# cwfparsonson/ddls

Hardware: AMD Instinct MI355X
Metric: ppo_env_steps_per_sec (higher is better)
Workload: dtype fp32; 1 GPU; model=pacml_gnn_msg32_hidden64_2rounds, global_batch=4096, seq_len=150, parallelism=dp1, ramp=4x4x2_32workers, envs_per_rank=256, env_engine=gpu_resident, num_sgd_iter=50, sgd_minibatch_size=128

## Files before the change

ddls_amd/ops/hip/cached_step.hip:

```cpp
#include <hip/hip_runtime.h>
#include <torch/extension.h>
#include <ATen/cuda/CUDAContext.h>
#include <cstdlib>
#include <cstring>
#include <vector>

#include "cs_stage.h"

#define LN_EPS 1e-5f

#define FMA(a, b, c) __builtin_fmaf((a), (b), (c))
__device__ __forceinline__ float mul_rn(float a, float b) {
  float p = a * b;
  asm("" : "+v"(p));
  return p;
}

#define KF0 5
#define KFE 2
#define KH 16
#define KMSG 32
#define KHID 64
#define KOUT 16
#define KGF 34
// ... 1709 lines not shown
      const float surr1 = ratio * A_b, surr2 = r_cl * A_b;
      float ds = ratio * A_b;
      if (surr2 < surr1 && (ratio < 1.f - D.clip || ratio > 1.f + D.clip))
        ds = 0.f;
      const float coef = -ds - klc;
      P.hent[b] = ent;
      P.coef[b] = coef;
      sHent[s] = ent;
      sCoef[s] = coef;
    }
    __syncthreads();
    for (int x = tid; x < ns * KA; x += NT) {
      const int s = x / KA, a = x % KA;
      const int b = c0 + s;
      const long u = (long)b * KA + a;
      const long act = P.actions[b];
      const float c = sCoef[s] / D.B;
      const float pj = sPp[s][a];
      const float lpj = sLp[s][a];
      P.p[u] = pj;
      P.lp[u] = lpj;
      const float delta = (a == (int)act) ? 1.f : 0.f;
      const float gl = mul_rn(c, delta - pj)
                       + mul_rn(mul_rn(D.ent_coef / D.B, pj),
                                lpj + sHent[s]);
      P.glogits[u] = gl;
      sGL[s][a] = gl;
    }
    if (tid >= 128 && tid < 128 + ns) {
      const int s = tid - 128;
      const int b = c0 + s;
      const float verr = sVal[s] - P.vtarg[b];
      const float mk = (verr * verr <= D.vf_clip) ? 1.f : 0.f;
      const float gv = D.vf_coef * 2.f * verr * mk / D.B;
      P.gvalue[b] = gv;
      sGV[s] = gv;
    }
    __syncthreads();
#pragma unroll
    for (int s = 0; s < HS; ++s) {
      if (s < ns) {
        const int j = tid;
        const long u = (long)(c0 + s) * KFC + j;
        float acc = 0.f;
#pragma unroll
        for (int a = 0; a < KA; ++a) {
          const float w = sW2p[a * HD_ROW + hd_pad(j)];
          if (a < 5) acc = FMA(w, sGL[s][a], acc);
          else acc = acc + mul_rn(w, sGL[s][a]);
        }
        const float gp = hp[s] > 0.f ? acc : 0.f;
        const float av = w2v * sGV[s];
        const float gv = hv[s] > 0.f ? av : 0.f;
        P.gh1p[u] = gp;
        P.gh1v[u] = gv;
        sGHp[s][j] = gp;
        sGHv[s][j] = gv;
      }
    }
    __syncthreads();
    for (int x = tid; x < ns * KFIN; x += NT) {
      const int s = x / KFIN, i = x % KFIN;
      float acc = 0.f;
#pragma unroll 8
      for (int j = 0; j < KFC; ++j) {
        acc = FMA(sW1p[j * KFIN + i], sGHp[s][j], acc);
        acc = FMA(sW1v[j * KFIN + i], sGHv[s][j], acc);
      }
      P.gfinal[(long)(c0 + s) * KFIN + i] = acc;
      sGF[s][i] = acc;
    }
    __syncthreads();
    for (int x = tid; x < ns * KGF; x += NT) {
      const int s = x / KGF, i = x % KGF;
      float acc = 0.f;
#pragma unroll
      for (int o = 0; o < KGE; ++o)
        acc = acc + mul_rn(sWg[o * KGF + i], sGF[s][KOUT + o]);
      P.gu34[(long)(c0 + s) * KGF + i] = acc;
    }
  }
}

__global__ void __launch_bounds__(256)
cs_fwd_comb2_pool_kernel(CachedPtrs P, CachedDims D) {
  constexpr int PT = 256;
  __shared__ float sH2[PT * KOUT];
  const int tid = threadIdx.x;
  const int m = blockIdx.x;
  const long lo = P.model_nptr[m], hi = P.model_nptr[m + 1];
  float acc = 0.f;
  for (long v0 = lo; v0 < hi; v0 += PT) {
    const long v1 = min(hi, v0 + PT);
    __syncthreads();
    for (long x = tid; x < (v1 - v0) * KOUT; x += 256) {
      const long v = v0 + x / KOUT;
      const int i = (int)(x % KOUT);
      const long qlo = P.indptr[v], qhi = P.indptr[v + 1];
      float out = 0.f;
      if (qhi > qlo) {
        float a = P.rs2[v * KOUT + i];
        for (long q = qlo; q < qhi; ++q)
          a = a + P.re2[P.order[q] * KOUT + i];
        out = a / (float)(qhi - qlo + 1);
      }
      P.h2[v * KOUT + i] = out;
      sH2[x] = out;
    }
    __syncthreads();
    if (tid < KOUT)
      for (long v = v0; v < v1; ++v) acc = acc + sH2[(v - v0) * KOUT + tid];
  }
  if (tid < KOUT) P.pooled[(long)m * KOUT + tid] = acc / (float)(hi - lo);
}

template <int L>
__global__ void __launch_bounds__(ROW_NT)
cs_fwd_comb1_mlp2_lanes_kernel(CachedPtrs P, CachedDims D) {
  constexpr int RPB = ROW_NT / L;
  const int nbN = (D.N + RPB - 1) / RPB;
  if ((int)blockIdx.x < nbN) {
    const long r0 = (long)blockIdx.x * RPB;
    rows_fwd_lanes<KHID, KH, 0, L>(
        P, W_LN_N2_W, r0, D.N,
        [&](long v, int i) {
          const long lo = P.indptr[v], hi = P.indptr[v + 1];
          float out = 0.f;
          if (hi > lo) {
            float acc = P.rs1[v * KHID + i];
            for (long q = lo; q < hi; ++q)
              acc = acc + P.re1[P.order[q] * KHID + i];
            out = acc / (float)(hi - lo + 1);
          }
          P.h1[v * KHID + i] = out;
          return out;
        },
        P.xh_h2, P.rst_h2, P.hn2);
  } else {
    const long r0 = (long)(blockIdx.x - nbN) * RPB;
    rows_fwd_lanes<KFE, KH, 0, L>(
        P, W_LN_E2_W, r0, D.E,
        [&](long k, int i) { return P.e[k * KFE + i]; },
        P.xh_e2, P.rst_e2, P.he2);
  }
}

template <int L>
__global__ void __launch_bounds__(ROW_NT)
cs_bwd_scat2_mlp2_lanes_kernel(CachedPtrs P, CachedDims D) {
  constexpr int RPB = ROW_NT / L;
  const int nbN = (D.N + RPB - 1) / RPB;
  if ((int)blockIdx.x < nbN) {
    const long r0 = (long)blockIdx.x * RPB;
    rows_bwd_lanes<KHID, KH, KH, 0, L, true>(
        P, W_LN_N2_W, r0, D.N,
        [&](long v, int o) {
          const long lo = P.src_indptr[v], hi = P.src_indptr[v + 1];
          float acc = P.gms2[v * KMSG + o];
          for (long q = lo; q < hi; ++q)
            acc = acc + P.gme2[P.src_order[q] * KMSG + o];
          P.ghn2[v * KH + o] = acc;
          return acc;
        },
        P.hn2, P.xh_h2, P.rst_h2, P.gpn1, P.gu_h2, P.gh1b);
  } else {
    const long r0 = (long)(blockIdx.x - nbN) * RPB;
// ... 385 lines not shown
          }
        }
#pragma unroll
        for (int q = 0; q < MYU2; ++q) {
          int u = tid + q * NT;
          if (u < KA * JW) {
            int a = u / JW, j = u % JW;
            float s = acc2[q];
            if (rt == TILE_K) {
#pragma unroll
              for (int t = 0; t < TILE_K; ++t) {
                if (t < 20) s = FMA(tGL[r0 + t][a], tHp[r0 + t][j], s);
                else s = s + mul_rn(tGL[r0 + t][a], tHp[r0 + t][j]);
              }
            } else {
              for (int t = 0; t < rt; ++t)
                s = FMA(tGL[r0 + t][a], tHp[r0 + t][j], s);
            }
            acc2[q] = s;
          }
        }
      }
      if (cj >= 0 && cj < JW) {
        if (st == WFC_ST) {
#pragma unroll 16
          for (int t = 0; t < WFC_ST; ++t) {
            bp = bp + tGp[t][cj];
            bv = bv + tGv[t][cj];
            w2v = FMA(tGV[t], tHv[t][cj], w2v);
          }
        } else {
          for (int t = 0; t < st; ++t) {
            bp = bp + tGp[t][cj];
            bv = bv + tGv[t][cj];
            w2v = FMA(tGV[t], tHv[t][cj], w2v);
          }
        }
      }
      if (jb == 0) {
        if (tid >= 128 && tid < 128 + KA) {
          if (st == WFC_ST) {
#pragma unroll 16
            for (int t = 0; t < WFC_ST; ++t) b2 = b2 + tGL[t][tid - 128];
          } else {
            for (int t = 0; t < st; ++t) b2 = b2 + tGL[t][tid - 128];
          }
        }
        if (tid == 128 + KA) {
          if (st == WFC_ST) {
#pragma unroll 16
            for (int t = 0; t < WFC_ST; ++t) b2 = b2 + tGV[t];
          } else {
            for (int t = 0; t < st; ++t) b2 = b2 + tGV[t];
          }
        }
      }
      __syncthreads();
    }
#pragma unroll
    for (int q = 0; q < MYU; ++q) {
      int u = tid + q * NT;
      if (u < JW * KFIN) {
        int j = u / KFIN, i = u % KFIN;
        WG_(W_P1_W)[(long)(j0 + j) * KFIN + i] = accp[q];
        WG_(W_V1_W)[(long)(j0 + j) * KFIN + i] = accv[q];
      }
    }
#pragma unroll
    for (int q = 0; q < MYU2; ++q) {
      int u = tid + q * NT;
      if (u < KA * JW) {
        int a = u / JW, j = u % JW;
        WG_(W_P2_W)[(long)a * KFC + j0 + j] = acc2[q];
      }
    }
    if (cj >= 0 && cj < JW) {
      WG_(W_P1_B)[j0 + cj] = bp;
      WG_(W_V1_B)[j0 + cj] = bv;
      WG_(W_V2_W)[j0 + cj] = w2v;
    }
    if (jb == 0) {
      if (tid >= 128 && tid < 128 + KA) WG_(W_P2_B)[tid - 128] = b2;
      if (tid == 128 + KA) WG_(W_V2_B)[0] = b2;
    }
  }
}

static_assert(CS_STAGE_THREADS == ROW_NT, "stage role runs a ROW_NT block");

template <int L>
__global__ void __launch_bounds__(ROW_NT)
cs_fwd_stage_mlp1_lanes_kernel(CachedPtrs P, CachedDims D, StagePtrs SP,
                               StageDims SD) {
  if (blockIdx.x == 0) {
    cs_stage_body(SP, SD);
    return;
  }
  constexpr int RPB = ROW_NT / L;
  const int blk = (int)blockIdx.x - 1;
  const int nbN = (D.N + RPB - 1) / RPB;
  if (blk < nbN) {
    const long r0 = (long)blk * RPB;
    rows_fwd_lanes<KF0, KH, 1, L>(
        P, W_LN_N1_W, r0, D.N,
        [&](long v, int i) { return P.z0[v * KF0 + i]; },
        P.xh_z1, P.rst_z1, P.hn1);
  } else {
    const long r0 = (long)(blk - nbN) * RPB;
    rows_fwd_lanes<KFE, KH, 0, L>(
        P, W_LN_E1_W, r0, D.E,
        [&](long k, int i) { return P.e[k * KFE + i]; },
        P.xh_e1, P.rst_e1, P.he1);
  }
}


template <int Din, int NF>
__device__ __forceinline__ float mod1_elem(
    const float* __restrict__ x, const float* __restrict__ gam,
    const float* __restrict__ bet, const float* __restrict__ w, float b,
    int c, float* __restrict__ xh_c, float* __restrict__ rstd_out) {
  float s = 0.f;
#pragma unroll
  for (int i = 0; i < Din; ++i) s = s + x[i];
  const float mu = s / Din;
  float var;
  {
    const float d0 = x[0] - mu;
    var = d0 * d0;
  }
#pragma unroll
  for (int i = 1; i < Din; ++i) {
    const float d = x[i] - mu;
    if (i >= Din - NF) var = FMA(d, d, var);
    else var = var + d * d;
  }
  float rstd;
  if ((Din & (Din - 1)) == 0) rstd = rsqrtf(FMA(var, 1.f / Din, LN_EPS));
  else rstd = rsqrtf(var / Din + LN_EPS);
  *rstd_out = rstd;
  *xh_c = (x[c] - mu) * rstd;
  float acc = b;
#pragma unroll
  for (int i = 0; i < Din; ++i) {
    const float xh = (x[i] - mu) * rstd;
    acc = FMA(FMA(xh, gam[i], bet[i]), w[i], acc);
  }
  return acc > 0.f ? acc : 0.f;
}

template <int L, bool EDGE>
__device__ __forceinline__ void mlp1_red1_rows(const CachedPtrs& P, long r0,
                                               long nrows) {
  constexpr int RPB = ROW_NT / L;
  constexpr int XS = KMSG + 1;
  constexpr int RW = EDGE ? KF0 + KFE : KF0;
  constexpr int NSM = 2 * KMSG + KHID + (2 * KF0 + KH * KF0 + KH)
                      + (EDGE ? 2 * KFE + KH * KFE + KH : 0);
  constexpr int WQ = KMSG * KHID / ROW_NT;
  static_assert(RPB * RW <= ROW_NT && NSM <= 2 * ROW_NT
                && KMSG * KHID % ROW_NT == 0, "one staging pass");
  __shared__ float sGam[KMSG], sBet[KMSG], sW[KHID * XS], sB[KHID];
  __shared__ float sX[RPB * XS], sU[RPB * XS];
  __shared__ float sM1[2 * KF0 + KH * KF0 + KH + 2 * KFE + KH * KFE + KH];
  __shared__ float sIn[RPB * (KF0 + KFE)];
  float* const sGamN = sM1;
// ... 373 lines not shown
    }
    __syncthreads();
    const int ng = (D.B + SG_SPB - 1) / SG_SPB;
    for (int x = tid; x < ng * 4; x += ROW_NT) {
      const int g = x / 4, k = x % 4;
      const int b_lo = g * SG_SPB;
      const int nb = min(D.B - b_lo, SG_SPB);
      float acc = sT[b_lo][k];
      for (int t = 1; t < nb; ++t) acc = acc + sT[b_lo + t][k];
      sAcc[g][k] = acc;
    }
    __syncthreads();
    if (tid == 0) {
      const float inv = 1.f / D.B;
      const float klc = P.kl[0];
      for (int g = 0; g < ng; ++g) {
        const float pl = sAcc[g][0] * inv;
        const float vf = sAcc[g][1] * inv;
        const float kl = sAcc[g][2] * inv;
        const float ent = sAcc[g][3] * inv;
        atomicAdd(&P.stats[0], pl);
        atomicAdd(&P.stats[1], vf);
        atomicAdd(&P.stats[2], kl);
        atomicAdd(&P.stats[3], ent);
        atomicAdd(&P.stats[4],
                  FMA(-D.ent_coef, ent, FMA(D.vf_coef, vf, FMA(kl, klc, pl))));
      }
    }
  } else if ((int)blockIdx.x < nbN) {
    const long r0 = (long)blockIdx.x * SG_RPB;
    const long v = r0 + r;
    float g = 0.f;
    if (v < D.N) {
      const long lo = P.src_indptr[v], hi = P.src_indptr[v + 1];
      float acc = P.gms1[v * KMSG + i];
      for (long q = lo; q < hi; ++q)
        acc = acc + P.gme1[P.src_order[q] * KMSG + i];
      g = P.hn1[v * KH + i] > 0.f ? acc : 0.f;
      P.ghn1[v * KH + i] = g;
    }
    sG[r][i] = g;
    __syncthreads();
    for (int x = tid; x < SG_RPB * KF0; x += ROW_NT) {
      const int rr = x / KF0, ii = x % KF0;
      if (r0 + rr < D.N) {
        float acc = 0.f;
#pragma unroll
        for (int o = 0; o < KH; ++o)
          acc = FMA(sWN[o * KF0 + ii], sG[rr][o], acc);
        P.gu_z1[(r0 + rr) * KF0 + ii] = acc;
      }
    }
  } else {
    const long r0 = (long)(blockIdx.x - nbN) * SG_RPB;
    const long k = r0 + r;
    float g = 0.f;
    if (k < D.E) {
      const float ge = P.gme1[k * KMSG + KH + i];
      g = P.he1[k * KH + i] > 0.f ? ge : 0.f;
      P.ghe1[k * KH + i] = g;
    }
    sG[r][i] = g;
    __syncthreads();
    for (int x = tid; x < SG_RPB * KFE; x += ROW_NT) {
      const int rr = x / KFE, ii = x % KFE;
      if (r0 + rr < D.E) {
        float acc = 0.f;
#pragma unroll
        for (int o = 0; o < KH; ++o)
          acc = FMA(sWE[o * KFE + ii], sG[rr][o], acc);
        P.gu_e1[(r0 + rr) * KFE + ii] = acc;
      }
    }
  }
}


struct RowCfg {
  bool thread;
  int lanes;
  bool fused;
  bool overlap;
  bool merge;
};

static RowCfg row_cfg() {
  RowCfg c;
  const char* rk = getenv("DDLS_AMD_ROW_KERNELS");
  c.thread = (rk != nullptr && strcmp(rk, "thread") == 0);
  TORCH_CHECK(rk == nullptr || rk[0] == '\0' || c.thread
              || strcmp(rk, "lanes") == 0,
              "cached_step: DDLS_AMD_ROW_KERNELS must be 'thread' or "
              "'lanes', got '", rk, "'");
  c.lanes = 0;
  const char* rl = getenv("DDLS_AMD_ROW_LANES");
  if (rl != nullptr && rl[0] != '\0') {
    c.lanes = atoi(rl);
    TORCH_CHECK(c.lanes == 8 || c.lanes == 16 || c.lanes == 32,
                "cached_step: DDLS_AMD_ROW_LANES must be 8, 16 or 32, got '",
                rl, "'");
  }
  const char* sf = getenv("DDLS_AMD_STEP_FUSION");
  const bool off = (sf != nullptr && strcmp(sf, "off") == 0);
  TORCH_CHECK(sf == nullptr || sf[0] == '\0' || off || strcmp(sf, "on") == 0,
              "cached_step: DDLS_AMD_STEP_FUSION must be 'on' or 'off', got '",
              sf, "'");
  c.fused = !off && !c.thread;
  const char* so = getenv("DDLS_AMD_STEP_OVERLAP");
  const bool ooff = (so != nullptr && strcmp(so, "off") == 0);
  TORCH_CHECK(so == nullptr || so[0] == '\0' || ooff || strcmp(so, "on") == 0,
              "cached_step: DDLS_AMD_STEP_OVERLAP must be 'on' or 'off', got '",
              so, "'");
  c.overlap = !ooff && c.fused;
  const char* sm = getenv("DDLS_AMD_STEP_MERGE");
  const bool moff = (sm != nullptr && strcmp(sm, "off") == 0);
  TORCH_CHECK(sm == nullptr || sm[0] == '\0' || moff || strcmp(sm, "on") == 0,
              "cached_step: DDLS_AMD_STEP_MERGE must be 'on' or 'off', got '",
              sm, "'");
  c.merge = !moff && c.overlap;
  return c;
}

#define LAUNCH_ROWS(KERNEL_L, DEFL, rows0, rows1)                            \
  do {                                                                       \
    const int L_ = R.lanes ? R.lanes : (DEFL);                               \
    const int rpb_ = ROW_NT / L_;                                            \
    const int nb_ = ((rows0) + rpb_ - 1) / rpb_ + ((rows1) + rpb_ - 1) / rpb_; \
    if (nb_ > 0) {                                                           \
      if (L_ == 8)                                                           \
        hipLaunchKernelGGL(KERNEL_L(8), dim3(nb_), dim3(ROW_NT), 0, stream,  \
                           P, D);                                            \
      else if (L_ == 16)                                                     \
        hipLaunchKernelGGL(KERNEL_L(16), dim3(nb_), dim3(ROW_NT), 0, stream, \
                           P, D);                                            \
      else                                                                   \
        hipLaunchKernelGGL(KERNEL_L(32), dim3(nb_), dim3(ROW_NT), 0, stream, \
                           P, D);                                            \
    }                                                                        \
  } while (0)
#define K_FWD_MLP1(L) (cs_fwd_mlp_lanes_kernel<1, L>)
#define K_FWD_MLP2(L) (cs_fwd_mlp_lanes_kernel<2, L>)
#define K_FWD_RED1(L) (cs_fwd_reduce_lanes_kernel<1, L>)
#define K_FWD_RED2(L) (cs_fwd_reduce_lanes_kernel<2, L>)
#define K_BWD_RED1(L) (cs_bwd_reduce_lanes_kernel<1, L>)
#define K_BWD_RED2(L) (cs_bwd_reduce_lanes_kernel<2, L>)
#define K_BWD_MLP2(L) (cs_bwd_mlp2_lanes_kernel<L>)
#define K_FWD_COMB1_MLP2(L) (cs_fwd_comb1_mlp2_lanes_kernel<L>)
#define K_BWD_SCAT2_MLP2(L) (cs_bwd_scat2_mlp2_lanes_kernel<L>)

static void fill_ptrs(CachedPtrs& P, CachedDims& D, RowCfg& R,
                      std::vector<torch::Tensor>& T,
                      std::vector<double>& fs) {
  TORCH_CHECK((int)T.size() == C_NT, "cached_step: tensor list size ",
              T.size(), " != ", (int)C_NT);
  D.N = (int)T[C_Z0].size(0);
  D.F0 = (int)T[C_Z0].size(1);
  D.E = (int)T[C_E].size(0);
  D.FE = (int)T[C_E].size(1);
  D.M = (int)T[C_MODEL_NPTR].size(0) - 1;
  D.B = (int)T[C_GF].size(0);
  D.GFin = (int)T[C_GF].size(1);
  D.A = (int)T[C_MASK].size(1);
  D.H = (int)T[C_HN1].size(1);
  D.MSG = 2 * D.H;
  D.HID = (int)T[C_H1].size(1);
  D.OUT = (int)T[C_H2].size(1);
  D.GEMB = (int)T[C_FINAL].size(1) - D.OUT;
  D.FIN = (int)T[C_FINAL].size(1);
  D.FC = (int)T[C_H1P].size(1);
  const char* wm = getenv("DDLS_AMD_WGRAD_MFMA");
  D.wgrad_mfma = (wm != nullptr && wm[0] == '1') ? 1 : 0;
  R = row_cfg();
  D.clip = (float)fs[0];
  D.vf_clip = (float)fs[1];
  D.vf_coef = (float)fs[2];
  D.ent_coef = (float)fs[3];
  TORCH_CHECK(D.F0 == KF0 && D.FE == KFE && D.H == KH && D.MSG == KMSG
              && D.HID == KHID && D.OUT == KOUT && D.GFin == KGF
              && D.GEMB == KGE && D.FIN == KFIN && D.FC == KFC && D.A == KA,
              "cached_step: compiled for the tuned PAC-ML dims only");
  P.z0 = T[C_Z0].data_ptr<float>();
  P.e = T[C_E].data_ptr<float>();
  P.src = T[C_SRC].data_ptr<long>();
  P.dst = T[C_DST].data_ptr<long>();
  P.order = T[C_ORDER].data_ptr<long>();
  P.indptr = T[C_INDPTR].data_ptr<long>();
  P.src_order = T[C_SRC_ORDER].data_ptr<long>();
  P.src_indptr = T[C_SRC_INDPTR].data_ptr<long>();
  P.node_model = T[C_NODE_MODEL].data_ptr<long>();
  P.model_nptr = T[C_MODEL_NPTR].data_ptr<long>();
  P.model_ids = T[C_MODEL_IDS].data_ptr<long>();
  P.gf = T[C_GF].data_ptr<float>();
  P.mask = T[C_MASK].data_ptr<float>();
  P.actions = T[C_ACTIONS].data_ptr<long>();
  P.old_logp = T[C_OLD_LOGP].data_ptr<float>();
  P.adv = T[C_ADV].data_ptr<float>();
  P.vtarg = T[C_VTARG].data_ptr<float>();
  P.kl = T[C_KL].data_ptr<float>();
  P.flat_p = T[C_FLAT_P].data_ptr<float>();
  P.flat_g = T[C_FLAT_G].data_ptr<float>();
  P.offs = T[C_OFFS].data_ptr<long>();
  P.hn1 = T[C_HN1].data_ptr<float>();
// ... 61 lines not shown
  P.gu_h2 = T[C_GU_H2].data_ptr<float>();
  P.gu_e2 = T[C_GU_E2].data_ptr<float>();
  P.gu_m1e = T[C_GU_M1E].data_ptr<float>();
  P.gu_m1s = T[C_GU_M1S].data_ptr<float>();
  P.gu_z1 = T[C_GU_Z1].data_ptr<float>();
  P.gu_e1 = T[C_GU_E1].data_ptr<float>();
  P.wg_scratch = T[C_WG_SCRATCH].data_ptr<float>();
  TORCH_CHECK(T[C_WG_SCRATCH].numel() >= (long)6 * WSPLIT * WG_JSTRIDE,
              "cached_step: wg_scratch too small");
}

static void step_fwd_launches(const CachedPtrs& P, const CachedDims& D,
                              const RowCfg& R, const StagePtrs* SP,
                              const StageDims* SD) {
  hipStream_t stream = at::cuda::getCurrentCUDAStream();
  const int rows_b = (D.N + D.E + 255) / 256;
  const int comb1_b = ((long)D.N * D.HID + 255) / 256;
  const int comb2_b = ((long)D.N * D.OUT + 255) / 256;
  if (R.thread) {
    hipLaunchKernelGGL(cs_fwd_mlp_kernel<1>, dim3(rows_b), dim3(256), 0,
                       stream, P, D);
    hipLaunchKernelGGL(cs_fwd_reduce_kernel<1>, dim3(rows_b), dim3(256), 0,
                       stream, P, D);
  } else if (R.merge) {
    const int L_ = R.lanes ? R.lanes : 32;
    const int rpb_ = ROW_NT / L_;
    const int stage = SP != nullptr ? 1 : 0;
    const dim3 grid(stage + (D.E + rpb_ - 1) / rpb_ + (D.N + rpb_ - 1) / rpb_);
    StagePtrs sp0;
    StageDims sd0;
    memset(&sp0, 0, sizeof(sp0));
    memset(&sd0, 0, sizeof(sd0));
    const StagePtrs& sp = stage ? *SP : sp0;
    const StageDims& sd = stage ? *SD : sd0;
    if (grid.x > 0) {
      if (L_ == 8)
        hipLaunchKernelGGL(cs_fwd_stage_mlp1_red1_lanes_kernel<8>, grid,
                           dim3(ROW_NT), 0, stream, P, D, sp, sd, stage);
      else if (L_ == 16)
        hipLaunchKernelGGL(cs_fwd_stage_mlp1_red1_lanes_kernel<16>, grid,
                           dim3(ROW_NT), 0, stream, P, D, sp, sd, stage);
      else
        hipLaunchKernelGGL(cs_fwd_stage_mlp1_red1_lanes_kernel<32>, grid,
                           dim3(ROW_NT), 0, stream, P, D, sp, sd, stage);
    }
  } else {
    if (SP != nullptr) {
      const int L_ = R.lanes ? R.lanes : 16;
      const int rpb_ = ROW_NT / L_;
      const dim3 grid(1 + (D.N + rpb_ - 1) / rpb_ + (D.E + rpb_ - 1) / rpb_);
      if (L_ == 8)
        hipLaunchKernelGGL(cs_fwd_stage_mlp1_lanes_kernel<8>, grid,
                           dim3(ROW_NT), 0, stream, P, D, *SP, *SD);
      else if (L_ == 16)
        hipLaunchKernelGGL(cs_fwd_stage_mlp1_lanes_kernel<16>, grid,
                           dim3(ROW_NT), 0, stream, P, D, *SP, *SD);
      else
        hipLaunchKernelGGL(cs_fwd_stage_mlp1_lanes_kernel<32>, grid,
                           dim3(ROW_NT), 0, stream, P, D, *SP, *SD);
    } else {
      LAUNCH_ROWS(K_FWD_MLP1, 16, D.N, D.E);
    }
    LAUNCH_ROWS(K_FWD_RED1, 32, D.E, D.N);
  }
  if (!R.fused)
    hipLaunchKernelGGL(cs_fwd_combine_kernel<1>, dim3(comb1_b), dim3(256), 0,
                       stream, P, D);
  if (R.thread) {
    hipLaunchKernelGGL(cs_fwd_mlp_kernel<2>, dim3(rows_b), dim3(256), 0,
                       stream, P, D);
    hipLaunchKernelGGL(cs_fwd_reduce_kernel<2>, dim3(rows_b), dim3(256), 0,
                       stream, P, D);
  } else {
    if (R.fused)
      LAUNCH_ROWS(K_FWD_COMB1_MLP2, 16, D.N, D.E);
    else
      LAUNCH_ROWS(K_FWD_MLP2, 16, D.N, D.E);
    LAUNCH_ROWS(K_FWD_RED2, 16, D.E, D.N);
  }
  if (R.fused) {
    if (D.M > 0)
      hipLaunchKernelGGL(cs_fwd_comb2_pool_kernel, dim3(D.M), dim3(256), 0,
                         stream, P, D);
    const int hb = D.B < 32 ? D.B : 32;
    if (hb > 0)
      hipLaunchKernelGGL(cs_head_kernel, dim3(hb), dim3(256), 0, stream,
                         P, D);
    return;
  }
  hipLaunchKernelGGL(cs_fwd_combine_kernel<2>, dim3(comb2_b), dim3(256), 0,
                     stream, P, D);
  hipLaunchKernelGGL(cs_fwd_pool_kernel, dim3(1), dim3(512), 0, stream,
                     P, D);
  int head_blocks = ((long)D.B * D.FC + 255) / 256;
  if (head_blocks > 128) head_blocks = 128;
  hipLaunchKernelGGL(cs_fwd_head_kernel, dim3(head_blocks), dim3(256), 0,
                     stream, P, D);
  hipLaunchKernelGGL(cs_fwd_logits_kernel, dim3(D.B), dim3(512), 0,
                     stream, P, D);
  hipLaunchKernelGGL(cs_fwd_loss_kernel, dim3((D.B + 31) / 32), dim3(256),
                     0, stream, P, D);
}

void cached_step_fwd(std::vector<torch::Tensor> T, std::vector<double> fs) {
  CachedPtrs P;
  CachedDims D;
  RowCfg R;
  fill_ptrs(P, D, R, T, fs);
  step_fwd_launches(P, D, R, nullptr, nullptr);
}

void cached_step_fwd_staged(std::vector<torch::Tensor> T,
                            std::vector<double> fs,
                            std::vector<torch::Tensor> store,
                            torch::Tensor perm, torch::Tensor cursor,
                            torch::Tensor err,
                            std::vector<torch::Tensor> dims) {
  CachedPtrs P;
  CachedDims D;
  RowCfg R;
  fill_ptrs(P, D, R, T, fs);
  TORCH_CHECK(R.overlap, "cached_step_fwd_staged: needs the lane-parallel "
              "fused launches with DDLS_AMD_STEP_OVERLAP on");
  StagePtrs SP;
  StageDims SD;
  cs_stage_args(SP, SD, "cached_step_fwd_staged", store,
                {T[C_GF], T[C_MASK], T[C_MODEL_IDS], T[C_ACTIONS],
                 T[C_OLD_LOGP], T[C_ADV], T[C_VTARG]},
                perm, cursor, err, dims);
  step_fwd_launches(P, D, R, &SP, &SD);
}

bool cached_step_reduce_deferred(bool defer_reduce) {
  const char* wm = getenv("DDLS_AMD_WGRAD_MFMA");
  const bool mfma = (wm != nullptr && wm[0] == '1');
  return defer_reduce && row_cfg().merge && !mfma;
}

std::vector<int64_t> cached_step_fold_segments(std::vector<int64_t> offs) {
  TORCH_CHECK((int)offs.size() == W_COUNT, "cached_step_fold_segments: ",
              (int)W_COUNT, " slot offsets expected, got ", offs.size());
  const int din[6] = {KF0, KFE, KMSG, KHID, KFE, KMSG};
  const int dout[6] = {KH, KH, KHID, KH, KH, KOUT};
  const int slot[6] = {W_LN_N1_W, W_LN_E1_W, W_LN_R1_W,
                       W_LN_N2_W, W_LN_E2_W, W_LN_R2_W};
  std::vector<int64_t> segs;
  for (int j = 0; j < 6; ++j) {
    const int64_t base = (int64_t)j * WSPLIT * WG_JSTRIDE;
    const int64_t units = (int64_t)din[j] * dout[j];
    const int64_t quad[4][3] = {
        {offs[slot[j] + 2], units, base},
        {offs[slot[j] + 3], dout[j], base + units},
        {offs[slot[j]], din[j], base + units + dout[j]},
        {offs[slot[j] + 1], din[j], base + units + dout[j] + din[j]}};
    for (int q = 0; q < 4; ++q)
      for (int c = 0; c < 3; ++c) segs.push_back(quad[q][c]);
  }
  segs.push_back(WSPLIT);
  segs.push_back(WG_JSTRIDE);
  return segs;
}

void cached_step_bwd(std::vector<torch::Tensor> T, std::vector<double> fs,
                     bool defer_reduce) {
  CachedPtrs P;
  CachedDims D;
  RowCfg R;
  fill_ptrs(P, D, R, T, fs);
  hipStream_t stream = at::cuda::getCurrentCUDAStream();
  TORCH_CHECK(D.B <= 1024 && D.B <= SG_MAXB,
              "cached_step: minibatch larger than 1024");
  int hb = D.B < 32 ? D.B : 32;
  const int rows_b = (D.N + D.E + 255) / 256;
  const int scat_b = ((long)(D.N + D.E) * D.H + 255) / 256;
  if (!R.fused)
    hipLaunchKernelGGL(cs_bwd_head_kernel, dim3(hb), dim3(256), 0, stream,
                       P, D);
  if (R.overlap)
    hipLaunchKernelGGL(cs_bwd_pool_wfc_kernel, dim3(D.M + 1 + WFC_NFC),
                       dim3(256), 0, stream, P, D);
  else
    hipLaunchKernelGGL(cs_bwd_pool_kernel, dim3(1), dim3(512), 0, stream,
                       P, D);
  if (R.thread)
    hipLaunchKernelGGL(cs_bwd_reduce_kernel<2>, dim3(rows_b), dim3(256), 0,
                       stream, P, D);
  else
    LAUNCH_ROWS(K_BWD_RED2, 16, D.E, D.N);
  if (!R.fused)
    hipLaunchKernelGGL(cs_bwd_scatter_kernel<2>, dim3(scat_b), dim3(256), 0,
                       stream, P, D);
  if (R.thread) {
    hipLaunchKernelGGL(cs_bwd_mlp2_kernel, dim3(rows_b), dim3(256), 0,
                       stream, P, D);
    hipLaunchKernelGGL(cs_bwd_reduce_kernel<1>, dim3(rows_b), dim3(256), 0,
                       stream, P, D);
  } else {
    if (R.fused)
      LAUNCH_ROWS(K_BWD_SCAT2_MLP2, 16, D.N, D.E);
    else
      LAUNCH_ROWS(K_BWD_MLP2, 16, D.N, D.E);
    LAUNCH_ROWS(K_BWD_RED1, 32, D.E, D.N);
  }
  const int nsplit = D.wgrad_mfma ? 1 : WSPLIT;
  if (R.merge && nsplit > 1 && D.B > 0) {
    const int sg_b = (D.N + SG_RPB - 1) / SG_RPB + (D.E + SG_RPB - 1) / SG_RPB
                     + 1;
    hipLaunchKernelGGL(cs_bwd_scat1_gu1_w_kernel, dim3(sg_b + 6 * WSPLIT),
                       dim3(ROW_NT), 0, stream, P, D);
    if (!defer_reduce)
      hipLaunchKernelGGL(cs_bwd_w_reduce_kernel, dim3(6), dim3(256), 0,
                         stream, P, D);
    return;
  }
  if (R.fused) {
    const int sg_b = (D.N + SG_RPB - 1) / SG_RPB + (D.E + SG_RPB - 1) / SG_RPB
                     + 1;
    if (D.B > 0)
      hipLaunchKernelGGL(cs_bwd_scat1_gu1_kernel, dim3(sg_b), dim3(ROW_NT),
                         0, stream, P, D);
  } else {
    hipLaunchKernelGGL(cs_bwd_scatter_kernel<1>, dim3(scat_b), dim3(256), 0,
                       stream, P, D);
  }
  if (R.fused) {
  } else if (R.thread) {
    hipLaunchKernelGGL(cs_bwd_gu1_kernel, dim3(rows_b), dim3(256), 0, stream,
                       P, D);
  } else {
    const int gu1_b =
        (int)(((long)D.N * KF0 + (long)D.E * KFE + ROW_NT - 1) / ROW_NT);
    if (gu1_b > 0)
      hipLaunchKernelGGL(cs_bwd_gu1_lanes_kernel, dim3(gu1_b), dim3(ROW_NT),
                         0, stream, P, D);
  }
  hipLaunchKernelGGL(cs_bwd_w_kernel,
                     dim3(6 * nsplit + (R.overlap ? 0 : 1 + 16)), dim3(256),
                     0, stream, P, D);
  if (nsplit > 1 && !(defer_reduce && R.merge))
    hipLaunchKernelGGL(cs_bwd_w_reduce_kernel, dim3(6), dim3(256), 0,
                       stream, P, D);
}
```

Before: 23580 env_steps/s.

## Add wider-grid head and transposed-tile pool/weight-grad kernels behind HEAD flag

Adds a new fused head kernel that processes one sample per block and launches up to 128 blocks instead of 32, keeping per-thread first-layer weights in registers and using float4 LDS reads for the input-gradient reduction. Adds a new backward pool/weight-gradient kernel that splits the FC weight gradient into narrower column groups (more blocks), stages batch tiles transposed in LDS, and reads them with float4 vector loads. Both are enabled by default through a new DDLS_AMD_STEP_HEAD switch. The aim is more parallelism and cheaper LDS traffic in the head and weight-gradient phases, at the cost of more redundant weight loading per block and new 16-byte alignment requirements.

```diff
diff --git a/ddls_amd/ops/hip/cached_step.hip b/ddls_amd/ops/hip/cached_step.hip
--- a/ddls_amd/ops/hip/cached_step.hip
+++ b/ddls_amd/ops/hip/cached_step.hip
@@ -1815,6 +1815,288 @@
   }
 }
 
+#define HD2_WS (KFC + 4)
+#define HD2_MAXB 128
+#define LDS4(p) (*reinterpret_cast<const float4*>(p))
+__global__ void __launch_bounds__(256)
+cs_head2_kernel(CachedPtrs P, CachedDims D) {
+  constexpr int HS = 1;
+  __shared__ float sW2p[KA * HD_ROW];
+  __shared__ __align__(16) float sW1p[KFIN * HD2_WS], sW1v[KFIN * HD2_WS];
+  __shared__ float sWg[KGE * KGF];
+  __shared__ float sB2p[KA];
+  __shared__ float sGL[HS][KA], sGV[HS], sGF[HS][KFIN];
+  __shared__ __align__(16) float sGHp[HS][HD2_WS], sGHv[HS][HD2_WS];
+  __shared__ float sFin[HS][KFIN], sHp[HS][HD_ROW], sVred[HS][KFC];
+  __shared__ float sGf[HS][KGF], sU34[HS][KGF];
+  __shared__ float sGamG[KGF], sBetG[KGF], sBg[KGE];
+  __shared__ float sPart[HS][KA][16 + 1];
+  __shared__ float sRow[HS][KA], sPp[HS][KA], sLp[HS][KA];
+  __shared__ float sVal[HS], sCoef[HS], sHent[HS];
+  const int tid = threadIdx.x;
+  constexpr int NT = 256;
+  for (int x = tid; x < KA * KFC; x += NT)
+    sW2p[(x / KFC) * HD_ROW + hd_pad(x % KFC)] = WP(W_P2_W)[x];
+  for (int x = tid; x < KGE * KGF; x += NT) sWg[x] = WP(W_G_W)[x];
+  if (tid < KA) sB2p[tid] = WP(W_P2_B)[tid];
+  if (tid < KGF) {
+    sGamG[tid] = WP(W_LN_G_W)[tid];
+    sBetG[tid] = WP(W_LN_G_B)[tid];
+  }
+  if (tid < KGE) sBg[tid] = WP(W_G_B)[tid];
+  float w1p[KFIN], w1v[KFIN];
+#pragma unroll
+  for (int i = 0; i < KFIN; ++i) {
+    w1p[i] = WP(W_P1_W)[tid * KFIN + i];
+    w1v[i] = WP(W_V1_W)[tid * KFIN + i];
+  }
+#pragma unroll
+  for (int i = 0; i < KFIN; ++i) {
+    sW1p[i * HD2_WS + tid] = w1p[i];
+    sW1v[i * HD2_WS + tid] = w1v[i];
+  }
+  const float b1p = WP(W_P1_B)[tid], b1v = WP(W_V1_B)[tid];
+  const float w2v = WP(W_V2_W)[tid];
+  const float b2v = WP(W_V2_B)[0];
+  const float klc = P.kl[0];
+  const int wv = tid >> 6, ln = tid & 63;
+  const int per = (D.B + gridDim.x - 1) / gridDim.x;
+  const int b0 = blockIdx.x * per;
+  const int b1 = min(D.B, b0 + per);
+  for (int c0 = b0; c0 < b1; c0 += HS) {
+    const int ns = min(HS, b1 - c0);
+    const int xr_ = min(tid, ns * KA - 1);
+    const float r_mask = P.mask[(long)c0 * KA + xr_];
+    const long r_act = P.actions[c0 + xr_ / KA];
+    const int bw_ = c0 + min(wv, ns - 1);
+    const long w_act = P.actions[bw_];
+    const float w_old_lp = P.old_logp[bw_];
+    const float w_adv = P.adv[bw_];
+    const float r_vtarg = P.vtarg[c0 + min(max(tid - 128, 0), ns - 1)];
+    for (int x = tid; x < ns * KGF; x += NT)
+      sGf[x / KGF][x % KGF] = P.gf[(long)c0 * KGF + x];
+    for (int x = tid; x < ns * KOUT; x += NT) {
+      const int s = x / KOUT, i = x % KOUT;
+      const long mid = P.model_ids[c0 + s];
+      const float pv = P.pooled[mid * KOUT + i];
+      sFin[s][i] = pv;
+      P.fin[(long)(c0 + s) * KFIN + i] = pv;
+    }
+    const float fmin = -3.402823466e+38f;
+    float r_lm = logf(r_mask);
+    if (!(r_lm > fmin)) r_lm = fmin;
+    __syncthreads();
+    for (int x = tid; x < ns * KGF; x += NT) {
+      const int s = x / KGF, i = x % KGF;
+      const float* __restrict__ xr = sGf[s];
+      float sum = 0.f;
+#pragma unroll
+      for (int k = 0; k < KGF; ++k) sum = sum + xr[k];
+      const float mu = sum / KGF;
+      float var;
+      {
+        const float d0 = xr[0] - mu;
+        var = d0 * d0;
+      }
+#pragma unroll
+      for (int k = 1; k < KGF; ++k) {
+        const float d = xr[k] - mu;
+        var = var + d * d;
+      }
+      const float rstd = rsqrtf(var / KGF + LN_EPS);
+      const float xh = (xr[i] - mu) * rstd;
+      P.xh34[(long)(c0 + s) * KGF + i] = xh;
+      sU34[s][i] = FMA(xh, sGamG[i], sBetG[i]);
+    }
+    __syncthreads();
+    for (int x = tid; x < ns * KGE; x += NT) {
+      const int s = x / KGE, o = x % KGE;
+      float acc = sBg[o];
+#pragma unroll
+      for (int i = 0; i < KGF; ++i)
+        acc = FMA(sWg[o * KGF + i], sU34[s][i], acc);
+      sFin[s][KOUT + o] = acc;
+      P.fin[(long)(c0 + s) * KFIN + KOUT + o] = acc;
+    }
+    __syncthreads();
+    float hp[HS], hv[HS];
+#pragma unroll
+    for (int s = 0; s < HS; ++s) {
+      hp[s] = 0.f;
+      hv[s] = 0.f;
+      if (s < ns) {
+        float ap = b1p, av = b1v;
+#pragma unroll
+        for (int i = 0; i < KFIN; ++i) {
+          ap = FMA(w1p[i], sFin[s][i], ap);
+          av = FMA(w1v[i], sFin[s][i], av);
+        }
+        ap = ap > 0.f ? ap : 0.f;
+        av = av > 0.f ? av : 0.f;
+        const long u = (long)(c0 + s) * KFC + tid;
+        P.h1p[u] = ap;
+        P.h1v[u] = av;
+        hp[s] = ap;
+        hv[s] = av;
+        sHp[s][hd_pad(tid)] = ap;
+        sVred[s][tid] = w2v * av;
+      }
+    }
+    __syncthreads();
+    for (int x = tid; x < ns * KA * 16; x += NT) {
+      const int s = x / (KA * 16), r = x % (KA * 16);
+      const int a = r / 16, c = r % 16;
+      const float* __restrict__ w = sW2p + a * HD_ROW + c * HD_CS;
+      const float* __restrict__ h = sHp[s] + c * HD_CS;
+      float acc = FMA(w[0], h[0], 0.f);
+#pragma unroll
+      for (int i = 1; i < 16; ++i) {
+        if (i < 4) acc = FMA(w[i], h[i], acc);
+        else acc = acc + w[i] * h[i];
+      }
+      sPart[s][a][c] = acc;
+    }
+    if (wv < ns) {
+      const float* __restrict__ vr = sVred[wv];
+      float a0 = vr[ln] + vr[ln + 128];
+      const float a1 = vr[ln + 64] + vr[ln + 192];
+      a0 = a0 + a1;
+#pragma unroll
+      for (int off = 32; off > 0; off >>= 1)
+        a0 = a0 + __shfl_down(a0, off, 64);
+      if (ln == 0) {
+        const float val = a0 + b2v;
+        sVal[wv] = val;
+        P.values[c0 + wv] = val;
+      }
+    }
+    __syncthreads();
+    if (tid < ns * KA) {
+      const int s = tid / KA, a = tid % KA;
+      float acc = sB2p[a];
+#pragma unroll
+      for (int c = 0; c < 16; ++c) acc = acc + sPart[s][a][c];
+      sRow[s][a] = acc + r_lm;
+    }
+    __syncthreads();
+    if (wv < ns && ln == 0) {
+      const int s = wv;
+      const int b = c0 + s;
+      const float* __restrict__ row = sRow[s];
+      float mx = -3.0e38f;
+#pragma unroll
+      for (int a = 0; a < KA; ++a) mx = fmaxf(mx, row[a]);
+      float Z = 0.f;
+#pragma unroll
+      for (int a = 0; a < KA; ++a) Z = Z + __expf(row[a] - mx);
+      const float lse = mx + __logf(Z);
+      float ent = 0.f;
+#pragma unroll
+      for (int a = 0; a < KA; ++a) {
+        const float lp = row[a] - lse;
+        const float e = __expf(lp);
+        sLp[s][a] = lp;
+        sPp[s][a] = e;
+        ent = FMA(-lp, e, ent);
+      }
+      const float logp_a = sLp[s][w_act];
+      const float ratio = __expf(logp_a - w_old_lp);
+      const float A_b = w_adv;
+      const float r_cl = fminf(fmaxf(ratio, 1.f - D.clip), 1.f + D.clip);
+      const float surr1 = ratio * A_b, surr2 = r_cl * A_b;
+      float ds = ratio * A_b;
+      if (surr2 < surr1 && (ratio < 1.f - D.clip || ratio > 1.f + D.clip))
+        ds = 0.f;
+      const float coef = -ds - klc;
+      P.hent[b] = ent;
+      P.coef[b] = coef;
+      sHent[s] = ent;
+      sCoef[s] = coef;
+    }
+    __syncthreads();
+    if (tid < ns * KA) {
+      const int s = tid / KA, a = tid % KA;
+      const int b = c0 + s;
+      const long u = (long)b * KA + a;
+      const float c = sCoef[s] / D.B;
+      const float pj = sPp[s][a];
+      const float lpj = sLp[s][a];
+      P.p[u] = pj;
+      P.lp[u] = lpj;
+      const float delta = (a == (int)r_act) ? 1.f : 0.f;
+      const float gl = mul_rn(c, delta - pj)
+                       + mul_rn(mul_rn(D.ent_coef / D.B, pj),
+                                lpj + sHent[s]);
+      P.glogits[u] = gl;
+      sGL[s][a] = gl;
+    }
+    if (tid >= 128 && tid < 128 + ns) {
+      const int s = tid - 128;
+      const int b = c0 + s;
+      const float verr = sVal[s] - r_vtarg;
+      const float mk = (verr * verr <= D.vf_clip) ? 1.f : 0.f;
+      const float gv = D.vf_coef * 2.f * verr * mk / D.B;
+      P.gvalue[b] = gv;
+      sGV[s] = gv;
+    }
+    __syncthreads();
+#pragma unroll
+    for (int s = 0; s < HS; ++s) {
+      if (s < ns) {
+        const int j = tid;
+        const long u = (long)(c0 + s) * KFC + j;
+        float acc = 0.f;
+#pragma unroll
+        for (int a = 0; a < KA; ++a) {
+          const float w = sW2p[a * HD_ROW + hd_pad(j)];
+          if (a < 5) acc = FMA(w, sGL[s][a], acc);
+          else acc = acc + mul_rn(w, sGL[s][a]);
+        }
+        const float gp = hp[s] > 0.f ? acc : 0.f;
+        const float av = w2v * sGV[s];
+        const float gv = hv[s] > 0.f ? av : 0.f;
+        P.gh1p[u] = gp;
+        P.gh1v[u] = gv;
+        sGHp[s][j] = gp;
+        sGHv[s][j] = gv;
+      }
+    }
+    __syncthreads();
+    if (tid < ns * KFIN) {
+      const int s = tid / KFIN, i = tid % KFIN;
+      const float* __restrict__ wp = sW1p + i * HD2_WS;
+      const float* __restrict__ wvv = sW1v + i * HD2_WS;
+      const float* __restrict__ gp = sGHp[s];
+      const float* __restrict__ gv = sGHv[s];
+      float acc = 0.f;
+#pragma unroll 4
+      for (int j = 0; j < KFC; j += 4) {
+        const float4 a = LDS4(wp + j), b = LDS4(wvv + j);
+        const float4 g = LDS4(gp + j), h = LDS4(gv + j);
+        acc = FMA(a.x, g.x, acc);
+        acc = FMA(b.x, h.x, acc);
+        acc = FMA(a.y, g.y, acc);
+        acc = FMA(b.y, h.y, acc);
+        acc = FMA(a.z, g.z, acc);
+        acc = FMA(b.z, h.z, acc);
+        acc = FMA(a.w, g.w, acc);
+        acc = FMA(b.w, h.w, acc);
+      }
+      P.gfinal[(long)(c0 + s) * KFIN + i] = acc;
+      sGF[s][i] = acc;
+    }
+    __syncthreads();
+    for (int x = tid; x < ns * KGF; x += NT) {
+      const int s = x / KGF, i = x % KGF;
+      float acc = 0.f;
+#pragma unroll
+      for (int o = 0; o < KGE; ++o)
+        acc = acc + mul_rn(sWg[o * KGF + i], sGF[s][KOUT + o]);
+      P.gu34[(long)(c0 + s) * KGF + i] = acc;
+    }
+  }
+}
+
 __global__ void __launch_bounds__(256)
 cs_fwd_comb2_pool_kernel(CachedPtrs P, CachedDims D) {
   constexpr int PT = 256;
@@ -2366,6 +2648,426 @@
     if (jb == 0) {
       if (tid >= 128 && tid < 128 + KA) WG_(W_P2_B)[tid - 128] = b2;
       if (tid == 128 + KA) WG_(W_V2_B)[0] = b2;
+    }
+  }
+}
+
+#define WFC2_JW 4
+#define WFC2_NFC (KFC / WFC2_JW)
+#define WFC2_TS (WFC_ST + 4)
+#define WFC2_LDS_POOL (2 * 1024 + WFC_ST * KOUT + KOUT + 16)
+#define WFC2_LDS_G (WFC2_TS * (KGE + 3 * KGF))
+#define WFC2_LDS_FC (WFC2_TS * (KFIN + 4 * WFC2_JW + KA + 1))
+#define WFC2_LDS (WFC2_LDS_G > WFC2_LDS_FC ? WFC2_LDS_G : WFC2_LDS_FC)
+static_assert(WFC2_LDS >= WFC2_LDS_POOL, "pool role LDS");
+static_assert(WFC2_LDS * 4 <= 64 * 1024, "cs_bwd_pool_wfc2: LDS over 64 KB");
+static_assert(WFC2_JW % 4 == 0 && KFC % WFC2_JW == 0, "whole float4 columns");
+static_assert(WFC2_JW * KFIN <= 256, "one weight unit a thread");
+static_assert(WFC_ST % 64 == 0 && SG_MAXB % WFC_ST == 0, "tiles of whole waves");
+static_assert(TILE_K == 32, "20 fused + 12 rounded terms a full tile");
+
+__global__ void __launch_bounds__(256)
+cs_bwd_pool_wfc2_kernel(CachedPtrs P, CachedDims D) {
+  __shared__ __align__(16) float lds[WFC2_LDS];
+  const int tid = threadIdx.x;
+  constexpr int NT = 256;
+  constexpr int TS = WFC2_TS;
+  const int bid = blockIdx.x;
+
+  if (bid < D.M) {
+    const int m = bid;
+    int* smid = reinterpret_cast<int*>(lds);
+    int* slist = smid + 1024;
+    float (*sG)[KOUT] = reinterpret_cast<float (*)[KOUT]>(lds + 2048);
+    float* sP = lds + 2048 + WFC_ST * KOUT;
+    int* send = reinterpret_cast<int*>(sP + KOUT);
+    const long lo = P.model_nptr[m], hi = P.model_nptr[m + 1];
+    for (int b = tid; b < D.B; b += NT) smid[b] = (int)P.model_ids[b];
+    float acc = 0.f;
+    int k = 0;
+    for (int t0 = 0; t0 < D.B; t0 += WFC_ST) {
+      const int bt = min(WFC_ST, D.B - t0);
+      float rG[WFC_ST * KOUT / NT];
+#pragma unroll
+      for (int q = 0; q < WFC_ST * KOUT / NT; ++q) {
+        const int x = min(tid + q * NT, bt * KOUT - 1);
+        rG[q] = P.gfinal[(long)(t0 + x / KOUT) * KFIN + x % KOUT];
+      }
+      __syncthreads();
+      if (t0 == 0 && tid < 64) {
+        int cnt = 0;
+        for (int b0 = 0; b0 < D.B; b0 += 64) {
+          const int b = b0 + tid;
+          const bool mine = b < D.B && smid[min(b, D.B - 1)] == m;
+          const unsigned long long bal = __ballot(mine);
+          if (mine) slist[cnt + __popcll(bal & ((1ull << tid) - 1ull))] = b;
+          cnt += __popcll(bal);
+          if (tid == 0 && ((b0 + 64) % WFC_ST == 0 || b0 + 64 >= D.B))
+            send[b0 / WFC_ST] = cnt;
+        }
+      }
+#pragma unroll
+      for (int q = 0; q < WFC_ST * KOUT / NT; ++q) {
+        const int x = tid + q * NT;
+        if (x < bt * KOUT) sG[x / KOUT][x % KOUT] = rG[q];
+      }
+      __syncthreads();
+      if (tid < KOUT) {
+        const int k1 = send[t0 / WFC_ST];
+#pragma unroll 4
+        for (; k < k1; ++k) acc += sG[slist[k] - t0][tid];
+      }
+    }
+    if (tid < KOUT) {
+      P.gpool[(long)m * KOUT + tid] = acc;
+      sP[tid] = acc;
+    }
+    __syncthreads();
+    const float nn = (float)(hi - lo);
+    for (long u = lo * KOUT + tid; u < hi * KOUT; u += NT)
+      P.gh2[u] = sP[u % KOUT] / nn;
+    return;
+  }
+
+  if (bid == D.M) {
+    float* tG = lds;
+    float* tU = tG + KGE * TS;
+    float* tXH = tU + KGF * TS;
+    float* tGU = tXH + KGF * TS;
+    const long o_gam = P.offs[W_LN_G_W], o_bet = P.offs[W_LN_G_B];
+    const long o_w = P.offs[W_G_W], o_b = P.offs[W_G_B];
+    const float* __restrict__ gam = P.flat_p + o_gam;
+    const float* __restrict__ bet = P.flat_p + o_bet;
+    constexpr int UNITS = KGE * KGF;
+    constexpr int MYU = (UNITS + 255) / 256;
+    float acc[MYU];
+#pragma unroll
+    for (int q = 0; q < MYU; ++q) acc[q] = 0.f;
+    float bacc = 0.f, lacc = 0.f;
+    for (int r0 = 0; r0 < D.B; r0 += WFC_ST) {
+      const int rt = min(WFC_ST, D.B - r0);
+      {
+        constexpr int CX = WFC_ST * KGF / NT;
+        static_assert(WFC_ST * KGE / 4 == NT && CX * NT == WFC_ST * KGF,
+                      "whole trips");
+        float rXH[CX], rGU[CX], rGam[CX], rBet[CX];
+        const int gx = min(tid, rt * (KGE / 4) - 1);
+        const float4 rG = *reinterpret_cast<const float4*>(
+            P.gfinal + (long)(r0 + gx / (KGE / 4)) * KFIN + KOUT
+            + 4 * (gx % (KGE / 4)));
+#pragma unroll
+        for (int k = 0; k < CX; ++k) {
+          const int x = min(tid + k * NT, rt * KGF - 1);
+          rXH[k] = P.xh34[(long)r0 * KGF + x];
+          rGU[k] = P.gu34[(long)r0 * KGF + x];
+          rGam[k] = gam[x % KGF];
+          rBet[k] = bet[x % KGF];
+        }
+        if (tid < rt * (KGE / 4)) {
+          const int t = tid / (KGE / 4), c = 4 * (tid % (KGE / 4));
+          tG[(c + 0) * TS + t] = rG.x;
+          tG[(c + 1) * TS + t] = rG.y;
+          tG[(c + 2) * TS + t] = rG.z;
+          tG[(c + 3) * TS + t] = rG.w;
+        }
+#pragma unroll
+        for (int k = 0; k < CX; ++k) {
+          const int x = tid + k * NT;
+          if (x < rt * KGF) {
+            const int t = x / KGF, i = x % KGF;
+            tU[i * TS + t] = FMA(rXH[k], rGam[k], rBet[k]);
+            tXH[i * TS + t] = rXH[k];
+            tGU[i * TS + t] = rGU[k];
+          }
+        }
+      }
+      __syncthreads();
+      const int rt4 = rt & ~3;
+#pragma unroll
+      for (int q = 0; q < MYU; ++q) {
+        int u = tid + q * 256;
+        if (u < UNITS) {
+          const float* go = tG + (u / KGF) * TS;
+          const float* ui = tU + (u % KGF) * TS;
+          float a = acc[q];
+          if (rt == WFC_ST) {
+#pragma unroll 8
+            for (int t = 0; t < WFC_ST; t += 4) {
+              const float4 g = LDS4(go + t), v = LDS4(ui + t);
+              a = FMA(g.x, v.x, a);
+              a = FMA(g.y, v.y, a);
+              a = FMA(g.z, v.z, a);
+              a = FMA(g.w, v.w, a);
+            }
+          } else {
+            for (int t = 0; t < rt4; t += 4) {
+              const float4 g = LDS4(go + t), v = LDS4(ui + t);
+              a = FMA(g.x, v.x, a);
+              a = FMA(g.y, v.y, a);
+              a = FMA(g.z, v.z, a);
+              a = FMA(g.w, v.w, a);
+            }
+            for (int t = rt4; t < rt; ++t) a = FMA(go[t], ui[t], a);
+          }
+          acc[q] = a;
+        }
+      }
+      if (tid >= 64 && tid < 64 + KGE) {
+        const float* go = tG + (tid - 64) * TS;
+        for (int t = 0; t < rt4; t += 4) {
+          const float4 g = LDS4(go + t);
+          bacc = bacc + g.x;
+          bacc = bacc + g.y;
+          bacc = bacc + g.z;
+          bacc = bacc + g.w;
+        }
+        for (int t = rt4; t < rt; ++t) bacc = bacc + go[t];
+      }
+      if (tid >= 128 && tid < 128 + KGF) {
+        const float* gu = tGU + (tid - 128) * TS;
+        const float* xh = tXH + (tid - 128) * TS;
+        for (int t = 0; t < rt4; t += 4) {
+          const float4 g = LDS4(gu + t), x = LDS4(xh + t);
+          lacc = lacc + mul_rn(g.x, x.x);
+          lacc = lacc + mul_rn(g.y, x.y);
+          lacc = lacc + mul_rn(g.z, x.z);
+          lacc = lacc + mul_rn(g.w, x.w);
+        }
+        for (int t = rt4; t < rt; ++t) lacc = lacc + mul_rn(gu[t], xh[t]);
+      }
+      if (tid >= 192 && tid < 192 + KGF) {
+        const float* gu = tGU + (tid - 192) * TS;
+        for (int t = 0; t < rt4; t += 4) {
+          const float4 g = LDS4(gu + t);
+          lacc = lacc + g.x;
+          lacc = lacc + g.y;
+          lacc = lacc + g.z;
+          lacc = lacc + g.w;
+        }
+        for (int t = rt4; t < rt; ++t) lacc = lacc + gu[t];
+      }
+      __syncthreads();
+    }
+#pragma unroll
+    for (int q = 0; q < MYU; ++q) {
+      int u = tid + q * 256;
+      if (u < UNITS) P.flat_g[o_w + u] = acc[q];
+    }
+    if (tid >= 64 && tid < 64 + KGE) P.flat_g[o_b + tid - 64] = bacc;
+    if (tid >= 128 && tid < 128 + KGF) P.flat_g[o_gam + tid - 128] = lacc;
+    if (tid >= 192 && tid < 192 + KGF) P.flat_g[o_bet + tid - 192] = lacc;
+    return;
+  }
+
+  {
+    constexpr int JW = WFC2_JW;
+    constexpr int PV = JW * KFIN;
+    constexpr int A2 = KA * JW;
+    constexpr int A2_T0 = PV <= 128 ? 128 : NT - A2;
+    constexpr int CS_N = 2 * JW;
+    constexpr int W2V_T0 = PV;
+    constexpr int B2_T0 = NT - 32;
+    static_assert(A2_T0 >= 0 && A2_T0 + A2 <= NT && W2V_T0 + JW <= NT
+                  && KA + 1 <= 32, "roles fit the block");
+    const int jb = bid - D.M - 1;
+    if (jb >= WFC2_NFC) return;
+    const int j0 = jb * JW;
+    float* tF = lds;
+    float* tGp = tF + KFIN * TS;
+    float* tGv = tGp + JW * TS;
+    float* tHp = tGv + JW * TS;
+    float* tHv = tHp + JW * TS;
+    float* tGL = tHv + JW * TS;
+    const long o_p1w = P.offs[W_P1_W], o_v1w = P.offs[W_V1_W];
+    const long o_p2w = P.offs[W_P2_W], o_p1b = P.offs[W_P1_B];
+    const long o_v1b = P.offs[W_V1_B], o_v2w = P.offs[W_V2_W];
+    const long o_p2b = P.offs[W_P2_B], o_v2b = P.offs[W_V2_B];
+    float ap = 0.f, av = 0.f, s2 = 0.f, cs = 0.f, w2v = 0.f, b2 = 0.f;
+    const bool is_pv = tid < PV;
+    const bool is_a2 = tid >= A2_T0 && tid < A2_T0 + A2;
+    const bool is_cs = tid < CS_N;
+    const bool is_w2v = tid >= W2V_T0 && tid < W2V_T0 + JW;
+    const bool is_b2 = jb == 0 && tid >= B2_T0 && tid < B2_T0 + KA + 1;
+    const int pj = tid / KFIN, pi = tid % KFIN;
+    const int aa = (tid - A2_T0) / JW, aj = (tid - A2_T0) % JW;
+    for (int s0 = 0; s0 < D.B; s0 += WFC_ST) {
+      const int st = min(WFC_ST, D.B - s0);
+      {
+        constexpr int CF = WFC_ST * KFIN / 4 / NT;
+        constexpr int CL = (WFC_ST * KA + NT - 1) / NT;
+        constexpr int Q = JW / 4;
+        static_assert(CF * NT * 4 == WFC_ST * KFIN && WFC_ST * Q <= NT
+                      && WFC_ST <= NT, "whole trips");
+        float4 rF[CF];
+        float rGL[CL];
+#pragma unroll
+        for (int k = 0; k < CF; ++k) {
+          const int x = min(tid + k * NT, st * (KFIN / 4) - 1);
+          rF[k] = *reinterpret_cast<const float4*>(
+              P.fin + (long)s0 * KFIN + 4 * x);
+        }
+        const int cx = min(tid, st * Q - 1);
+        const long cg = (long)(s0 + cx / Q) * KFC + j0 + 4 * (cx % Q);
+        const float4 rGp = *reinterpret_cast<const float4*>(P.gh1p + cg);
+        const float4 rGv = *reinterpret_cast<const float4*>(P.gh1v + cg);
+        const float4 rHp = *reinterpret_cast<const float4*>(P.h1p + cg);
+        const float4 rHv = *reinterpret_cast<const float4*>(P.h1v + cg);
+#pragma unroll
+        for (int k = 0; k < CL; ++k) {
+          const int x = min(tid + k * NT, st * KA - 1);
+          rGL[k] = P.glogits[(long)s0 * KA + x];
+        }
+        const float rGV = P.gvalue[s0 + min(tid, st - 1)];
+#pragma unroll
+        for (int k = 0; k < CF; ++k) {
+          const int x = tid + k * NT;
+          if (x < st * (KFIN / 4)) {
+            const int t = x / (KFIN / 4), c = 4 * (x % (KFIN / 4));
+            tF[(c + 0) * TS + t] = rF[k].x;
+            tF[(c + 1) * TS + t] = rF[k].y;
+            tF[(c + 2) * TS + t] = rF[k].z;
+            tF[(c + 3) * TS + t] = rF[k].w;
+          }
+        }
+        if (tid < st * Q) {
+          const int t = tid / Q, c = 4 * (tid % Q);
+          tGp[(c + 0) * TS + t] = rGp.x;
+          tGp[(c + 1) * TS + t] = rGp.y;
+          tGp[(c + 2) * TS + t] = rGp.z;
+          tGp[(c + 3) * TS + t] = rGp.w;
+          tGv[(c + 0) * TS + t] = rGv.x;
+          tGv[(c + 1) * TS + t] = rGv.y;
+          tGv[(c + 2) * TS + t] = rGv.z;
+          tGv[(c + 3) * TS + t] = rGv.w;
+          tHp[(c + 0) * TS + t] = rHp.x;
+          tHp[(c + 1) * TS + t] = rHp.y;
+          tHp[(c + 2) * TS + t] = rHp.z;
+          tHp[(c + 3) * TS + t] = rHp.w;
+          tHv[(c + 0) * TS + t] = rHv.x;
+          tHv[(c + 1) * TS + t] = rHv.y;
+          tHv[(c + 2) * TS + t] = rHv.z;
+          tHv[(c + 3) * TS + t] = rHv.w;
+        }
+#pragma unroll
+        for (int k = 0; k < CL; ++k) {
+          const int x = tid + k * NT;
+          if (x < st * KA) tGL[(x % KA) * TS + x / KA] = rGL[k];
+        }
+        if (tid < st) tGL[KA * TS + tid] = rGV;
+      }
+      __syncthreads();
+      const int st4 = st & ~3;
+      if (is_pv) {
+        const float* fr = tF + pi * TS;
+        const float* gp = tGp + pj * TS;
+        const float* gv = tGv + pj * TS;
+        if (st == WFC_ST) {
+#pragma unroll 8
+          for (int t = 0; t < WFC_ST; t += 4) {
+            const float4 f = LDS4(fr + t), a = LDS4(gp + t), b = LDS4(gv + t);
+            ap = FMA(a.x, f.x, ap);
+            av = FMA(b.x, f.x, av);
+            ap = FMA(a.y, f.y, ap);
+            av = FMA(b.y, f.y, av);
+            ap = FMA(a.z, f.z, ap);
+            av = FMA(b.z, f.z, av);
+            ap = FMA(a.w, f.w, ap);
+            av = FMA(b.w, f.w, av);
+          }
+        } else {
+          for (int t = 0; t < st4; t += 4) {
+            const float4 f = LDS4(fr + t), a = LDS4(gp + t), b = LDS4(gv + t);
+            ap = FMA(a.x, f.x, ap);
+            av = FMA(b.x, f.x, av);
+            ap = FMA(a.y, f.y, ap);
+            av = FMA(b.y, f.y, av);
+            ap = FMA(a.z, f.z, ap);
+            av = FMA(b.z, f.z, av);
+            ap = FMA(a.w, f.w, ap);
+            av = FMA(b.w, f.w, av);
+          }
+          for (int t = st4; t < st; ++t) {
+            ap = FMA(gp[t], fr[t], ap);
+            av = FMA(gv[t], fr[t], av);
+          }
+        }
+      }
+      if (is_a2) {
+        const float* gl = tGL + aa * TS;
+        const float* hp = tHp + aj * TS;
+        for (int r0 = 0; r0 < st; r0 += TILE_K) {
+          const int rt = min(TILE_K, st - r0);
+          if (rt == TILE_K) {
+#pragma unroll
+            for (int t = 0; t < TILE_K; t += 4) {
+              const float4 g = LDS4(gl + r0 + t), h = LDS4(hp + r0 + t);
+              if (t < 20) {
+                s2 = FMA(g.x, h.x, s2);
+                s2 = FMA(g.y, h.y, s2);
+                s2 = FMA(g.z, h.z, s2);
+                s2 = FMA(g.w, h.w, s2);
+              } else {
+                s2 = s2 + mul_rn(g.x, h.x);
+                s2 = s2 + mul_rn(g.y, h.y);
+                s2 = s2 + mul_rn(g.z, h.z);
+                s2 = s2 + mul_rn(g.w, h.w);
+              }
+            }
+          } else {
+            for (int t = 0; t < rt; ++t)
+              s2 = FMA(gl[r0 + t], hp[r0 + t], s2);
+          }
+        }
+      }
+      if (is_cs) {
+        const float* g = tGp + tid * TS;
+        for (int t = 0; t < st4; t += 4) {
+          const float4 v = LDS4(g + t);
+          cs = cs + v.x;
+          cs = cs + v.y;
+          cs = cs + v.z;
+          cs = cs + v.w;
+        }
+        for (int t = st4; t < st; ++t) cs = cs + g[t];
+      }
+      if (is_w2v) {
+        const float* gvl = tGL + KA * TS;
+        const float* hv = tHv + (tid - W2V_T0) * TS;
+        for (int t = 0; t < st4; t += 4) {
+          const float4 g = LDS4(gvl + t), h = LDS4(hv + t);
+          w2v = FMA(g.x, h.x, w2v);
+          w2v = FMA(g.y, h.y, w2v);
+          w2v = FMA(g.z, h.z, w2v);
+          w2v = FMA(g.w, h.w, w2v);
+        }
+        for (int t = st4; t < st; ++t) w2v = FMA(gvl[t], hv[t], w2v);
+      }
+      if (is_b2) {
+        const float* g = tGL + (tid - B2_T0) * TS;
+        for (int t = 0; t < st4; t += 4) {
+          const float4 v = LDS4(g + t);
+          b2 = b2 + v.x;
+          b2 = b2 + v.y;
+          b2 = b2 + v.z;
+          b2 = b2 + v.w;
+        }
+        for (int t = st4; t < st; ++t) b2 = b2 + g[t];
+      }
+      __syncthreads();
+    }
+    if (is_pv) {
+      P.flat_g[o_p1w + (long)(j0 + pj) * KFIN + pi] = ap;
+      P.flat_g[o_v1w + (long)(j0 + pj) * KFIN + pi] = av;
+    }
+    if (is_a2) P.flat_g[o_p2w + (long)aa * KFC + j0 + aj] = s2;
+    if (is_cs) {
+      if (tid < JW) P.flat_g[o_p1b + j0 + tid] = cs;
+      else P.flat_g[o_v1b + j0 + tid - JW] = cs;
+    }
+    if (is_w2v) P.flat_g[o_v2w + j0 + tid - W2V_T0] = w2v;
+    if (is_b2) {
+      if (tid - B2_T0 < KA) P.flat_g[o_p2b + tid - B2_T0] = b2;
+      else P.flat_g[o_v2b] = b2;
     }
   }
 }
@@ -2905,6 +3607,7 @@
   bool fused;
   bool overlap;
   bool merge;
+  bool head;
 };
 
 static RowCfg row_cfg() {
@@ -2941,6 +3644,12 @@
               "cached_step: DDLS_AMD_STEP_MERGE must be 'on' or 'off', got '",
               sm, "'");
   c.merge = !moff && c.overlap;
+  const char* sh = getenv("DDLS_AMD_STEP_HEAD");
+  const bool hoff = (sh != nullptr && strcmp(sh, "off") == 0);
+  TORCH_CHECK(sh == nullptr || sh[0] == '\0' || hoff || strcmp(sh, "on") == 0,
+              "cached_step: DDLS_AMD_STEP_HEAD must be 'on' or 'off', got '",
+              sh, "'");
+  c.head = !hoff && c.merge;
   return c;
 }
 
@@ -3168,10 +3877,16 @@
     if (D.M > 0)
       hipLaunchKernelGGL(cs_fwd_comb2_pool_kernel, dim3(D.M), dim3(256), 0,
                          stream, P, D);
-    const int hb = D.B < 32 ? D.B : 32;
-    if (hb > 0)
-      hipLaunchKernelGGL(cs_head_kernel, dim3(hb), dim3(256), 0, stream,
-                         P, D);
+    const int hb = R.head ? (D.B < HD2_MAXB ? D.B : HD2_MAXB)
+                          : (D.B < 32 ? D.B : 32);
+    if (hb > 0) {
+      if (R.head)
+        hipLaunchKernelGGL(cs_head2_kernel, dim3(hb), dim3(256), 0, stream,
+                           P, D);
+      else
+        hipLaunchKernelGGL(cs_head_kernel, dim3(hb), dim3(256), 0, stream,
+                           P, D);
+    }
     return;
   }
   hipLaunchKernelGGL(cs_fwd_combine_kernel<2>, dim3(comb2_b), dim3(256), 0,
@@ -3262,7 +3977,15 @@
   if (!R.fused)
     hipLaunchKernelGGL(cs_bwd_head_kernel, dim3(hb), dim3(256), 0, stream,
                        P, D);
-  if (R.overlap)
+  if (R.head) {
+    for (const float* q : {(const float*)P.fin, (const float*)P.gfinal,
+                           (const float*)P.gh1p, (const float*)P.gh1v,
+                           (const float*)P.h1p, (const float*)P.h1v})
+      TORCH_CHECK(reinterpret_cast<uintptr_t>(q) % 16 == 0,
+                  "cached_step: head scratch tensors must be 16-byte aligned");
+    hipLaunchKernelGGL(cs_bwd_pool_wfc2_kernel, dim3(D.M + 1 + WFC2_NFC),
+                       dim3(256), 0, stream, P, D);
+  } else if (R.overlap)
     hipLaunchKernelGGL(cs_bwd_pool_wfc_kernel, dim3(D.M + 1 + WFC_NFC),
                        dim3(256), 0, stream, P, D);
   else
```

After: 26260 env_steps/s, median of 6. 1.11x the previous value.
